# neozenith/sqlite-muninn

Measured on AMD Instinct MI355X. Metric: kNN queries/sec (10k-query batch, k=10, ef=128, 1M x 768 f32 HNSW index) + recall@10, higher is better.
Workload: dtype f32

## Files before the change

### include/muninn_hip.h

```cpp
#ifndef MUNINN_HIP_H
#define MUNINN_HIP_H

#include <stddef.h>
#include <stdint.h>

#ifdef __cplusplus
extern "C" {
#endif

#define MN_ABI_VERSION 2

typedef enum { MN_METRIC_L2 = 0, MN_METRIC_COSINE = 1, MN_METRIC_INNER_PRODUCT = 2 } mn_metric;

typedef enum { MN_ORDER_SSE = 0, MN_ORDER_WAVE = 1 } mn_order;

typedef enum {
    MN_BUILD_SEQUENTIAL = 0,
    MN_BUILD_BATCHED = 1
} mn_build_mode;

typedef struct {
    int64_t id;
    float distance;
} mn_search_result;
// ... 44 lines not shown

int mn_hnsw_get_vector(mn_index *idx, int64_t id, float *out);

int mn_hnsw_node_count(mn_index *idx);
int64_t mn_hnsw_entry_point(mn_index *idx);
int mn_hnsw_max_level(mn_index *idx);
int mn_hnsw_node_level(mn_index *idx, int64_t id);
int mn_hnsw_node_deleted(mn_index *idx, int64_t id);
int mn_hnsw_neighbors(mn_index *idx, int64_t id, int level, int64_t *out, int cap);
int mn_hnsw_load_node(mn_index *idx, int64_t id, const float *vector, int level, int deleted);
int mn_hnsw_load_neighbors(mn_index *idx, int64_t id, int level, const int64_t *nbrs, int n);
int mn_hnsw_set_entry(mn_index *idx, int64_t entry_point, int max_level);

int mn_hnsw_slot_count(mn_index *idx);
int mn_hnsw_export_nodes(mn_index *idx, int64_t *ids, int *levels, int *deleted);
int mn_hnsw_export_vectors(mn_index *idx, float *out);
int mn_hnsw_row_width(mn_index *idx, int level);
int mn_hnsw_export_links(mn_index *idx, int level, int *out, int *width);

int64_t mn_hnsw_take_dirty(mn_index *idx, int64_t *ids, int64_t cap);

int64_t mn_hnsw_edges_of(mn_index *idx, const int64_t *ids, int n, int64_t *out_src, int64_t *out_dst, int *out_level,
                         float *out_dist, int64_t cap);

typedef struct {
    double last_kernel_ms;
    int64_t last_n_dist;
    int64_t last_n_expanded;
    int64_t last_n_overflow;
    int64_t last_n_exact_rows;
    int64_t last_n_rows_lanes4;
    int64_t last_n_rows_lanes8;
    int64_t last_n_rows_lanes16;
} mn_launch_stats;
int mn_hnsw_last_launch(mn_index *idx, mn_launch_stats *out);
typedef struct {
    double search_ms, link_ms;
    int64_t n_dist, n_expanded;
    int64_t batches, nodes;
} mn_build_stats;
int mn_hnsw_build_stats(mn_index *idx, mn_build_stats *out, int reset);
void *mn_dev_malloc(mn_index *idx, size_t bytes);
void mn_dev_free(mn_index *idx, void *p);
int mn_dev_upload(mn_index *idx, void *dst_dev, const void *src_host, size_t bytes);
int mn_dev_download(mn_index *idx, void *dst_host, const void *src_dev, size_t bytes);
int mn_hnsw_bruteforce_topk(mn_index *idx, const float *d_queries, int64_t nq, int k, int64_t *out_ids);

typedef struct {
    int64_t n_queries, n_mfma_queries, n_fallback_queries, n_rescored_rows, n_bound_violations;
    float kernel_ms;
} mn_exact_stats;
int mn_hnsw_search_exact_batch(mn_index *idx, const float *queries, int64_t nq, int k,
                               const int64_t *allow_ids, int64_t n_allow,
                               int64_t *out_ids, float *out_dists, int *out_counts);
int mn_hnsw_search_exact_batch_dev(mn_index *idx, const float *d_queries, int64_t nq, int k,
                                   const int64_t *allow_ids, int64_t n_allow,
                                   int64_t *d_out_ids, float *d_out_dists, int *d_out_counts);
int mn_hnsw_last_exact(mn_index *idx, mn_exact_stats *out);

int mn_hnsw_knn_graph(mn_index *idx, int k, float max_distance, int64_t *out_ids, float *out_dists, int *out_counts);
int mn_hnsw_knn_graph_dev(mn_index *idx, int k, float max_distance, int64_t *d_out_ids, float *d_out_dists, int *d_out_counts);

typedef struct {
    int32_t r1, r2;
    double weight;
} mn_er_edge;
// ... 168 lines not shown
```

### sqlite-muninn_amd/csrc/mn_beam.hpp

```cpp
#pragma once
#include "mn_dist.hpp"

template <bool COH> DEVI int ld_link(const int *p) {
    if (COH)
        return __hip_atomic_load(p, __ATOMIC_RELAXED, __HIP_MEMORY_SCOPE_AGENT);
    return *p;
}
DEVI void st_link(int *p, int v) { __hip_atomic_store(p, v, __ATOMIC_RELAXED, __HIP_MEMORY_SCOPE_AGENT); }


struct WHeap {
    uint2 *l;
    unsigned long long *g;
    int lcap, gcap;
    int size;
    int ovf;
    int sorted = 0;
};

DEVI uint2 hget(const WHeap &h, int i) {
    if (i < h.lcap)
        return h.l[i];
    unsigned long long v = __hip_atomic_load(&h.g[i - h.lcap], __ATOMIC_RELAXED, __HIP_MEMORY_SCOPE_AGENT);
    return make_uint2((unsigned)(v & 0xffffffffull), (unsigned)(v >> 32));
// ... 98 lines not shown
static __device__ unsigned long long mn_phase[MN_PHASE_N];
#define PH_DECL unsigned long long ph_t = __builtin_amdgcn_s_memrealtime()
#define PH_ADD(w, k)                                                                                                             \
    do {                                                                                                                         \
        const unsigned long long ph_n = __builtin_amdgcn_s_memrealtime();                                                        \
        (w).ph[k] += ph_n - ph_t;                                                                                                \
        ph_t = ph_n;                                                                                                             \
    } while (0)
#define PH_CNT(w, k, n) (w).ph[k] += (n)
#else
#define PH_DECL
#define PH_ADD(w, k)
#define PH_CNT(w, k, n)
#endif

struct WaveCtx {
#ifdef MN_PHASE_TIMING
    unsigned long long ph[MN_PHASE_N] = {0, 0, 0, 0, 0, 0, 0, 0, 0, 0, 0, 0, 0, 0, 0, 0};
#endif
    float *tile = nullptr;
    const float *q;
    float qnorm;
    int *scratch;
    unsigned long long n_dist, n_exp;
    int *rlog = nullptr;
    int rcap = 0, nr = 0;
    CoopCtx *coop = nullptr;
    int no_spec_rows = 0;
    int lp_on = 0;
    LoQuery lq = {0.0f, 0.0};
    unsigned long long n_skip = 0;
    int sv_lanes = 0;
    unsigned long long n_l8 = 0, n_l16 = 0;
};
DEVI bool getenv_spec_off(const WaveCtx &w) { return (w.no_spec_rows & 1) != 0; }

DEVI void log_row_read(const MnDevIndex &ix, WaveCtx &w, int node, int level, int lane) {
    if (!w.rlog)
        return;
    if (lane == 0 && w.nr < w.rcap) {
        int *e = w.rlog + (size_t)w.nr * MN_RLOG_INTS;
        e[0] = level == 0 ? node : -(ix.up_off[node] + level - 1) - 2;
        e[1] = (int)0xff800000u;
        e[2] = e[3] = -1;
        e[4] = 0;
    }
    w.nr++;
}
DEVI void log_greedy_detail(WaveCtx &w, float to_beat, int from, int moved_to, int lane) {
    if (!w.rlog)
        return;
    if (lane == 0 && w.nr >= 1 && w.nr <= w.rcap) {
        int *e = w.rlog + (size_t)(w.nr - 1) * MN_RLOG_INTS;
        e[1] = __float_as_int(to_beat);
        e[2] = from;
        e[3] = moved_to;
        e[4] = 1;
    }
}
DEVI void log_row_detail(WaveCtx &w, float worst, unsigned long long could_push, int lane, int kind = 0) {
    if (!w.rlog)
        return;
    if (lane == 0 && w.nr >= 1 && w.nr <= w.rcap) {
        int *e = w.rlog + (size_t)(w.nr - 1) * MN_RLOG_INTS;
        e[1] = __float_as_int(worst);
        e[2] = (int)(unsigned)(could_push & 0xffffffffull);
// ... 104 lines not shown
                    i0 = c0 + 64;
                    fresh = false;
                    continue;
                }
                if (LOG && !WIDE)
                    log_greedy_detail(w, cur_d, i0, -1, lane);
                break;
            }
            int c = __ffsll((long long)better) - 1;
            const float beaten = cur_d;
            const int from = i0;
            cur_d = __shfl(d, c);
            cur = __shfl(myslot, c);
            int pos_of_me = pos;
            __builtin_amdgcn_wave_barrier();
            if (valid)
                w.scratch[rank] = pos_of_me;
            __builtin_amdgcn_wave_barrier();
            i0 = w.scratch[c] + 1;
            i0 = rfl(i0);
            cur = rfl(cur);
            if (LOG && !WIDE)
                log_greedy_detail(w, beaten, from, i0 - 1, lane);
            changed = 1;
            fresh = true;
        }
    }
    return cur;
}

template <int ORDER, int NCH, bool COH = false, bool WIDE = false, bool LOG = false, bool LP = false>
DEVI void beam_layer(const MnDevIndex &ix, WaveCtx &w, WHeap &cand, WHeap &res, unsigned *bitmap, int entry, int level,
                     int ef, int lane) {
    cand.size = 0;
    res.size = 0;
    if (!(ix.has_deleted && ix.deleted[entry])) {
        float d = ctx_distance<ORDER, NCH>(ix, w, entry, 1, lane);
        d = __shfl(d, 0);
        w.n_dist += 1;
        heap_push(cand, entry, d, lane);
        heap_push(res, entry, -d, lane);
        if (lane == 0) {
            int vi = level == 0 ? entry : ix.up_off[entry];
            atomicOr(&bitmap[vi >> 5], 1u << (vi & 31));
        }
    }
    int patience_max = ef / 4;
    if (patience_max < 10)
        patience_max = 10;
    int stale = 0;
    int guard = 0;
    while (cand.size > 0 && guard < (1 << 24)) {
        guard++;
        PH_DECL;
        uint2 c = heap_pop(cand, lane);
        const float cd = u2f(c.x);
        if (res.size >= ef) {
            float worst = -u2f(rflu(hget(res, 1).x));
            if (cd > worst)
                break;
        }
        if (stale >= patience_max && res.size >= ef)
            break;
        const int node = (int)c.y;
        int W;
        const int *row = link_row(ix, node, level, W);
        w.n_exp++;
        if (LOG)
            log_row_read(ix, w, node, level, lane);
        PH_ADD(w, 0);
        PH_CNT(w, 5, 1);
        int improved = 0;
        const int nchunk = WIDE ? (W + 63) >> 6 : 1;
        for (int ch = 0; ch < nchunk; ch++) {
        const int c0 = WIDE ? ch << 6 : 0;
        int nb = (c0 + lane < W) ? ld_link<COH>(row + c0 + lane) : -1;
        bool todo = false;
        if (nb >= 0) {
            int vi = level == 0 ? nb : ix.up_off[nb];
            unsigned bit = 1u << (vi & 31);
            unsigned old = atomicOr(&bitmap[vi >> 5], bit);
            todo = !(old & bit) && !(ix.has_deleted && ix.deleted[nb]);
        }
        unsigned long long m = __ballot(todo);
        int n = __popcll(m);
        PH_ADD(w, 1);
        if (n > 0) {
            int rank = __popcll(m & ((1ull << lane) - 1ull));
            __builtin_amdgcn_wave_barrier();
            if (todo)
                w.scratch[rank] = nb;
            __builtin_amdgcn_wave_barrier();
            int myslot = lane < n ? w.scratch[lane] : 0;
            w.n_dist += n;
            int ne = n;
            if (LP && w.lp_on && res.size >= ef) {
                const float worst0 = -u2f(rflu(hget(res, 1).x));
                const float lb = lo_rows_bound(ix, w.q, w.lq, myslot, n, lane);
                const bool keep = lane < n && !(lb >= worst0);
                const unsigned long long km = __ballot(keep);
                ne = __popcll(km);
                if (ne < n) {
                    w.n_skip += n - ne;
                    const int kr = __popcll(km & ((1ull << lane) - 1ull));
                    __builtin_amdgcn_wave_barrier();
                    if (keep)
                        w.scratch[kr] = myslot;
                    __builtin_amdgcn_wave_barrier();
                    myslot = lane < ne ? w.scratch[lane] : 0;
                }
                PH_ADD(w, 8);
                PH_CNT(w, 9, ne == 0);
                PH_CNT(w, 10, ne >= 1 && ne <= 4);
                PH_CNT(w, 11, ne >= 5 && ne <= 8);
                PH_CNT(w, 12, ne >= 9 && ne <= 16);
                PH_CNT(w, 13, ne > 16);
                PH_CNT(w, 14, 1);
                PH_CNT(w, 15, n);
            }
            float d = 0.0f;
            int quads = 1;
            if (LP && ORDER == MN_ORDER_SSE_V && NCH == 1)
                quads = w.sv_lanes ? w.sv_lanes >> 2 : (ne <= 4 ? 4 : ne <= 8 ? 2 : 1);
            if (LP && quads > 1 && ne > 0) {
                d = rows_distance_spread(ix, w.q, w.qnorm, myslot, ne, lane, quads);
                if (quads == 4)
                    w.n_l16 += ne;
                else
                    w.n_l8 += ne;
            } else if (!LP || ne > 0) {
                int dl = lane;
                if (LP)
                    asm volatile("" : "+v"(dl));
                d = ctx_distance<ORDER, NCH>(ix, w, myslot, ne, dl);
            }
            PH_ADD(w, 2);
            unsigned long long am;
            float worst_log = __builtin_inff();
            if (res.size >= ef) {
                float worst0 = -u2f(rflu(hget(res, 1).x));
                am = __ballot(lane < ne && d < worst0);
                worst_log = worst0;
            } else {
                am = __ballot(lane < ne);
            }
            if (LOG && !WIDE && w.rlog)
                log_row_detail(w, worst_log, __ballot(todo && ((am >> rank) & 1ull)), lane, 2);
            PH_CNT(w, 4, __popcll(am));
            while (am) {
                int i = __ffsll((long long)am) - 1;
                am &= am - 1;
                float di = __shfl(d, i);
                int si = __shfl(myslot, i);
                di = u2f(rflu(f2u(di)));
                si = rfl(si);
                if (res.size < ef) {
                    heap_push(cand, si, di, lane);
                    heap_push(res, si, -di, lane);
                    improved = 1;
                } else {
                    float worst = -u2f(rflu(hget(res, 1).x));
                    if (di < worst) {
                        heap_push(cand, si, di, lane);
                        heap_pop(res, lane);
                        heap_push(res, si, -di, lane);
                        improved = 1;
                    }
                }
            }
            PH_ADD(w, 3);
        } else if (LOG && !WIDE && w.rlog) {
            log_row_detail(w, res.size >= ef ? -u2f(rflu(hget(res, 1).x)) : __builtin_inff(), 0ull, lane, 2);
        }
        }
        stale = improved ? 0 : stale + 1;
    }
    if (guard >= (1 << 24))
        cand.ovf = 1;
#ifdef MN_PHASE_TIMING
    if (lane == 0)
        for (int k = 0; k < MN_PHASE_N; k++) {
            atomicAdd(&mn_phase[k], w.ph[k]);
            w.ph[k] = 0;
        }
#endif
}




#define MN_SA_R 4
#define MN_SA_CAP (64 * MN_SA_R)
#define MN_SA_EACH(X) X(0, k0, v0, s0) X(1, k1, v1, s1) X(2, k2, v2, s2) X(3, k3, v3, s3)
#define MN_SA_DONE ((int)0x80000000)

struct SQueue {
    float k0, k1, k2, k3;
    int v0, v1, v2, v3;
    int rn;
    float wk;
};
// ... 286 lines not shown
```

### sqlite-muninn_amd/csrc/mn_device.hpp

```cpp
#pragma once
#include <hip/hip_runtime.h>
#include <stdint.h>
#include <stdlib.h>

#define MN_WAVE 64

typedef unsigned mn_lo_t;
#define MN_LO_BITS 10
#define MN_LO_CMAX 511
#define MN_LO_LINE_CODES 96
#define MN_LO_LINE_WORDS 32
struct __align__(16) MnLoMeta {
    float scale;
    float resid;
    float xn_lo;
    float xn_hi;
};
#define MN_LO_MIN_LD 192
__host__ __device__ inline bool mn_lo_enabled(int ld) { return ld >= MN_LO_MIN_LD && (ld & 63) == 0; }
__host__ __device__ inline int mn_lo_lines(int ld) { return (ld + MN_LO_LINE_CODES - 1) / MN_LO_LINE_CODES; }
__host__ __device__ inline size_t mn_lo_row_words(int ld) { return (size_t)mn_lo_lines(ld) * MN_LO_LINE_WORDS; }
__host__ __device__ inline int mn_lo_q_floats(int ld) { return mn_lo_enabled(ld) ? mn_lo_lines(ld) * MN_LO_LINE_CODES : ld; }
__host__ __device__ inline int mn_lo_code(unsigned w, int f) { return (int)(w << (32 - MN_LO_BITS * (f + 1))) >> (32 - MN_LO_BITS); }
__host__ __device__ inline unsigned mn_lo_pack(int c0, int c1, int c2) {
    return ((unsigned)c0 & 0x3ffu) | (((unsigned)c1 & 0x3ffu) << 10) | (((unsigned)c2 & 0x3ffu) << 20);
}
constexpr int MN_ORDER_SSE_V = 0;
constexpr int MN_ORDER_WAVE_V = 1;

struct MnDevIndex {
    const float *vectors;
    const float *norms;
    int *links0;
    int *links_up;
    const int *up_off;
    const signed char *levels;
    const unsigned char *deleted;
    unsigned char *dirty;
    const long long *ids;
    int dim, ld, metric, order;
    int W0, WU;
    int M0, MU;
    int WX;
    int n_slots;
    int n_pool_rows;
    int has_deleted;
    const mn_lo_t *vec_lo;
    const MnLoMeta *lo_meta;
};

#define MN_QC 6
struct MnSearchArgs {
    const float *queries;
    const int *query_slots;
    long long nq;
    int k;
    int ef;
    int entry_slot, max_level;
    long long *out_ids;
    float *out_dists;
    int *out_counts;
    int *sel;
    int *nsel;
    int nlev;
    const int *up_bm_index;
    unsigned *bitmap0;
    long long bm0_words;
    unsigned *bitmap_up;
    long long bmu_words;
    uint2 *cand_ovf;
    int cand_gcap;
    uint2 *res_ovf;
    int res_gcap;
    unsigned long long *counters;
    unsigned long long *q_counters;
    int use_tile;
    int lds_bitmap;
    int *readlog;
    int readcap;
    int *nread;
    int lat_tile_rows;
    unsigned lat_tile_off;
    int surv_lanes;
    int no_spec_rows;
};
size_t mn_lds_optin_limit();
bool mn_lds_grant(const void *kernel, size_t bytes);
template <typename K> inline bool mn_lds_grant_for(K kernel, size_t bytes) { return mn_lds_grant(reinterpret_cast<const void *>(kernel), bytes); }
inline int mn_no_spec_rows(long long n_slots, int ld) {
    const char *sr = getenv("MN_SPEC_ROWS");
    const bool big = (size_t)n_slots * ld * sizeof(float) > ((size_t)256 << 20);
    return sr ? (atoi(sr) == 0 ? 1 : 0) : (big ? 0 : 1);
}

#ifndef MN_CAND_LDS
#define MN_CAND_LDS 256
#endif
#ifndef MN_RES_LDS
#define MN_RES_LDS 256
#endif

void mn_module_touch_kernels();
void mn_module_touch_seq();
void mn_module_touch_spec();
void mn_module_touch_build();
void mn_launch_prep_rows(const MnDevIndex &ix, int first_slot, int n, float *norms_out, mn_lo_t *lo_out, MnLoMeta *meta_out,
                         hipStream_t st);
int mn_launch_dist_batch(int metric, int order, const float *d_query, const float *d_rows, long long n, int dim, int ld,
                         float *d_out, hipStream_t st);
size_t mn_dist_batch_lds_bytes(int ld);
size_t mn_search_lds_bytes(int ld, bool tile);
size_t mn_coop_lds_bytes(int ld, bool tile);
size_t mn_spec_commit_min_lds_bytes(int ld);
size_t mn_link_reverse_lds_bytes(int ld, int WX, int nq);
size_t mn_bruteforce_lds_bytes(int ld);
inline size_t mn_row_lds_bytes(int ld) { return (size_t)ld * sizeof(float); }
// ... 71 lines not shown
```

### sqlite-muninn_amd/csrc/mn_dist.hpp

```cpp
#pragma once
#include "mn_device.hpp"

#define DEVI __device__ __forceinline__

DEVI int rfl(int v) { return __builtin_amdgcn_readfirstlane(v); }
DEVI unsigned rflu(unsigned v) { return (unsigned)__builtin_amdgcn_readfirstlane((int)v); }
DEVI float u2f(unsigned u) { return __uint_as_float(u); }
DEVI unsigned f2u(float f) { return __float_as_uint(f); }
DEVI double rfl_f64(double v) {
    const unsigned long long b = (unsigned long long)__double_as_longlong(v);
    return __longlong_as_double((long long)(((unsigned long long)rflu((unsigned)(b >> 32)) << 32) | rflu((unsigned)b)));
}


DEVI float cosine_finish(float dot, float na, float nb) {
    float denom = __fmul_rn(sqrtf(na), sqrtf(nb));
    if (denom < 1e-30f)
        return 1.0f;
    return __fsub_rn(1.0f, __fdiv_rn(dot, denom));
}

DEVI float wave_butterfly(float acc) {
#pragma unroll
    for (int m = 32; m >= 1; m >>= 1)
// ... 609 lines not shown
}

template <int ORDER, int NCH, bool LAT = false>
DEVI float rows_distance(const MnDevIndex &ix, const float *q_lds, float qnorm, int myslot, int n, int lane,
                         float *tile = nullptr, int tile_rows = 0) {
    if (ix.metric == 0) {
        return rows_accumulate<ORDER, NCH, true, LAT>(ix, q_lds, myslot, n, lane, tile, tile_rows);
    }
    float dot = rows_accumulate<ORDER, NCH, false, LAT>(ix, q_lds, myslot, n, lane, tile, tile_rows);
    if (ix.metric == 2)
        return -dot;
    float nb = (lane < n) ? ix.norms[myslot] : 1.0f;
    return cosine_finish(dot, qnorm, nb);
}

DEVI float rows_distance_spread(const MnDevIndex &ix, const float *q_lds, float qnorm, int myslot, int n, int lane, int Q) {
    if (ix.metric == 0)
        return sse_rows_spread<true>(ix, q_lds, myslot, n, lane, Q);
    const float dot = sse_rows_spread<false>(ix, q_lds, myslot, n, lane, Q);
    if (ix.metric == 2)
        return -dot;
    const float nb = (lane < n) ? ix.norms[myslot] : 1.0f;
    return cosine_finish(dot, qnorm, nb);
}


DEVI float lo_deq(int c, float s) { return __fmul_rn((float)c, s); }
DEVI double mn_gamma(int n) {
    const double nu = (double)n * 0x1p-24;
    return nu / (1.0 - nu);
}

template <bool L2, int UB>
DEVI void lo_lines(const uint4 *__restrict__ row, const float *q, float s, int lines, int &k, float &acc) {
    for (; k + UB <= lines; k += UB) {
        uint4 v[UB];
#pragma unroll
        for (int u = 0; u < UB; u++)
            v[u] = row[8 * (k + u)];
        __builtin_amdgcn_sched_barrier(0);
#pragma unroll
        for (int u = 0; u < UB; u++) {
            const float4 qa = *reinterpret_cast<const float4 *>(q + MN_LO_LINE_CODES * (k + u));
            const float4 qb = *reinterpret_cast<const float4 *>(q + MN_LO_LINE_CODES * (k + u) + 4);
            const float4 qc = *reinterpret_cast<const float4 *>(q + MN_LO_LINE_CODES * (k + u) + 8);
            const float qe[12] = {qa.x, qa.y, qa.z, qa.w, qb.x, qb.y, qb.z, qb.w, qc.x, qc.y, qc.z, qc.w};
            const unsigned w4[4] = {v[u].x, v[u].y, v[u].z, v[u].w};
#pragma unroll
            for (int e = 0; e < 12; e++) {
                const float x = lo_deq(mn_lo_code(w4[e / 3], e % 3), s);
                if (L2) {
                    const float d = __fsub_rn(qe[e], x);
                    acc = fmaf(d, d, acc);
                } else {
                    acc = fmaf(qe[e], x, acc);
                }
            }
            __builtin_amdgcn_sched_barrier(0);
        }
    }
}

template <bool L2>
DEVI float lo_rows_accumulate(const MnDevIndex &ix, const float *q_lds, int myslot, float sc, int n, int lane) {
    float mine = 0.0f;
    int ln = lane;
    asm volatile("" : "+v"(ln));
    const int c = ln & 7, r = ln >> 3;
    const int lines = mn_lo_lines(ix.ld);
    const size_t row_words = mn_lo_row_words(ix.ld);
    for (int t = 0; t < n; t += 8) {
        const int rr = t + r < n ? t + r : n - 1;
        const int sl = __shfl(myslot, rr);
        const float s = __shfl(sc, rr);
        const uint4 *row = reinterpret_cast<const uint4 *>(ix.vec_lo + (size_t)sl * row_words) + c;
        const float *q = q_lds + 12 * c;
        float acc = 0.0f;
        int k = 0;
        lo_lines<L2, 8>(row, q, s, lines, k, acc);
        lo_lines<L2, 2>(row, q, s, lines, k, acc);
        lo_lines<L2, 1>(row, q, s, lines, k, acc);
        acc += quad_xor1(acc);
        acc += quad_xor2(acc);
        acc += __int_as_float(__builtin_amdgcn_ds_swizzle(__float_as_int(acc), 0x101F));
        const float got = __shfl(acc, ((ln - t) & 7) << 3);
        if (ln >= t && ln < t + 8)
            mine = got;
    }
    return mine;
}

struct LoQuery {
    double qs_lo;
    double qn_hi;
};
DEVI LoQuery lo_query(float qsq, int ld) {
    LoQuery lq;
    lq.qs_lo = sqrt((double)qsq) * (1.0 - 0x1p-40);
    const double lost = (double)ld * 0x1p-149;
    lq.qn_hi = sqrt(((double)qsq + lost) / (1.0 - 2.0 * mn_gamma(ld + 8))) * (1.0 + 0x1p-40);
    return lq;
}

DEVI float lo_lower_bound(int metric, float A, const MnLoMeta &m, const LoQuery &lq, int ld) {
    const double a = A, r = m.resid, g = mn_gamma(ld + 8), u = 0x1p-24;
    if (!(fabs(a) <= 3.0e38) || !(r <= 3.0e38))
        return -__builtin_inff();
    double lb;
    if (metric == 0) {
        const double l = (double)sqrtf((float)(fmax(a - (double)ld * 0x1p-147, 0.0) * (1.0 - 4.0 * g))) * (1.0 - 0x1p-21) - 2.0 * r;
        lb = l > 0.0 ? l * l * (1.0 - 4.0 * g) : 0.0;
    } else {
        const double e = 2.0 * (lq.qn_hi * (r + g * (2.0 * (double)m.xn_hi + r)) + (double)ld * 0x1p-147);
        if (metric == 2) {
            lb = -(a + e);
        } else {
            const double den = lq.qs_lo * (double)m.xn_lo * (1.0 - 8.0 * u);
            if (!(den >= 1e-28))
                return -__builtin_inff();
            lb = 1.0 - fmax(a + e, 0.0) / den * (1.0 + 4.0 * u);
        }
    }
    lb -= fabs(lb) * 0x1p-20 + 0x1p-120;
    const float f = __double2float_rd(lb);
    return f == f ? f : -__builtin_inff();
}

template <int ORDER>
DEVI float lds_self_norm(const float *q_lds, int dim, int ld, int lane) {
    if (ORDER == MN_ORDER_SSE_V) {
        float v = sse_row<false>(q_lds, q_lds, dim, lane);
        return __shfl(v, 0);
    }
    return wave_row_generic<false>(q_lds, q_lds, ld, lane);
}

DEVI float lo_rows_bound(const MnDevIndex &ix, const float *q_lds, const LoQuery &lq, int myslot, int n, int lane) {
    MnLoMeta m = {1.0f, __builtin_inff(), 0.0f, 0.0f};
    if (lane < n)
        m = ix.lo_meta[myslot];
    const float A = ix.metric == 0 ? lo_rows_accumulate<true>(ix, q_lds, myslot, m.scale, n, lane)
                                   : lo_rows_accumulate<false>(ix, q_lds, myslot, m.scale, n, lane);
    return lane < n ? lo_lower_bound(ix.metric, A, m, lq, ix.ld) : -__builtin_inff();
}
```

### sqlite-muninn_amd/csrc/mn_index_int.hpp

```cpp
#pragma once
#include "../../include/muninn_hip.h"
#include "mn_comm.hpp"
#include "mn_device.hpp"
#include "mn_guard.hpp"
#include "mn_host.hpp"

#include <algorithm>
#include <cstdlib>
#include <cstring>
#include <string>
#include <vector>

void set_err(const char *fmt, ...) __attribute__((format(printf, 1, 2)));
#define HIPCHK(expr) MN_HIPCHK(set_err, expr)

template <typename T> struct DevBuf {
    T *p = nullptr;
    size_t cap = 0;
    DevBuf() = default;
    DevBuf(const DevBuf &) = delete;
    DevBuf &operator=(const DevBuf &) = delete;
    ~DevBuf() { release(); }
    int reserve(size_t n, bool keep, hipStream_t st, int fill_byte = -1, size_t want = 0) {
        if (n <= cap)
// ... 70 lines not shown
    bool dev_links_all = false;
    std::vector<std::pair<int, int>> h_dirty_rows;
    std::vector<float> load_vecs;
    int load_first = -1;
    DevBuf<unsigned> ws_bm0, ws_bmu;
    DevBuf<uint2> ws_cand, ws_res;
    DevBuf<float> ws_q, ws_outd;
    DevBuf<long long> ws_outi;
    DevBuf<int> ws_outc, ws_qslots, ws_sel, ws_nsel, ws_upidx;
    DevBuf<int> lk_target, lk_src, lk_counters, lk_count, lk_fill, lk_binoff, lk_touched, lk_bins, lk_newrows;
    DevBuf<int> lk_rec, lk_rec_all, lk_cls;
    DevBuf<unsigned long long> ws_counters;
    DevBuf<int> ws_state;
    DevBuf<int> er_slot, er_level, er_nbr;
    DevBuf<float> er_dist;
    DevBuf<int> ws_readlog, ws_nread, ws_ncommit, d_stamp0, d_stampU, d_sidx0, d_sidxU, d_saved_rows, d_pre_act, d_pre_cnt, d_pre_row, d_spec_why;
    int spec_epoch = 0;
    std::vector<int> staged;
    DevBuf<int> d_staged;
    DevBuf<int> sh_sel, sh_nsel, sh_gcnt;
    DevBuf<int> ws_chlog;
    bool want_chlog = false;
    std::vector<int> h_chlog;
    std::vector<unsigned char> h_stale;
    int n_stale = 0;
    unsigned char *pin = nullptr;
    size_t pin_cap = 0;
    DevBuf<unsigned long long> sh_ovf;
    int sh_ovf_pending = 0;
    DevBuf<long long> sh_gids;
    DevBuf<float> sh_gd;
    long long last_spec_searched = 0;
    bool broken = false;
    mn_launch_stats last = {0, 0, 0, 0, 0, 0, 0, 0};
    mn_exact_stats last_exact = {0, 0, 0, 0, 0, 0.0f};
};

int use_device(mn_index *x);
MnDevIndex dev_view(mn_index *x);
int ht_find(const mn_index *x, int64_t id);
void ht_grow(mn_index *x);
int random_level(mn_index *x);
int host_add_node(mn_index *x, int64_t id, int level, int deleted);
int64_t first_table_full(const mn_index *x, int64_t n);
void mark_stale(mn_index *x, int slot);
struct InsertUndo {
    int first, node_count, max_level, n_pool_rows, old_cap = 0, grew_at = -1;
    unsigned rng;
    int64_t entry_id;
    std::vector<int> old_ht;
};
void undo_insert(mn_index *x, InsertUndo &u);
int sync_meta(mn_index *x);
int upload_vectors(mn_index *x, int first, const float *vecs, int n, bool src_on_device = false);
int pull_links(mn_index *x);
int push_links(mn_index *x);
unsigned char *pin_reserve(mn_index *x, size_t need);
#define MN_PIN_META 0
#define MN_PIN_IN 64
#define MN_PIN_OUT 96
#define MN_PIN_VEC 256
inline size_t pin_log_off(const mn_index *x) { return (MN_PIN_VEC + (size_t)x->ld * sizeof(float) + 63) & ~(size_t)63; }
inline size_t pin_insert_bytes(const mn_index *x) {
    return pin_log_off(x) + ((size_t)1 + (size_t)MN_CHLOG_CAP * MN_CHLOG_INTS) * sizeof(int);
}

inline int cand_gcap(int ef) { return 16 * ef + 1024; }
// ... 10 lines not shown
```

### sqlite-muninn_amd/csrc/mn_index_search.hip

```cpp
#include "mn_index_int.hpp"

#include <cstdio>


static int reserve_search_ws(mn_index *x, int64_t nq, int ef) {
    hipStream_t st = x->stream;
    if (x->ws_bm0.reserve((size_t)nq * bm0_words(x->n_slots), false, st)) return -1;
    if (x->ws_cand.reserve((size_t)nq * cand_gcap(ef), false, st)) return -1;
    if (x->ws_res.reserve((size_t)nq * res_gcap(ef), false, st)) return -1;
    if (x->ws_counters.reserve(8, false, st)) return -1;
    return 0;
}

int prepare_search_ws(mn_index *x, int64_t nq, int ef, MnSearchArgs &a, bool zero_counters, bool lds_bitmap_ok) {
    hipStream_t st = x->stream;
    a.bm0_words = bm0_words(x->n_slots);
    a.cand_gcap = cand_gcap(ef);
    a.res_gcap = res_gcap(ef);
    if (reserve_search_ws(x, nq, ef))
        return -1;
    a.lds_bitmap = lds_bitmap_ok && nq <= 128 &&
                   (long long)mn_search_lds_bytes(x->ld, true) + 1024 + a.bm0_words * (long long)sizeof(unsigned) <= 64 * 1024 &&
                   !(getenv("MN_COOP") && atoi(getenv("MN_COOP")) == 0) && !(getenv("MN_LDS_BITMAP") && atoi(getenv("MN_LDS_BITMAP")) == 0);
    if (!a.lds_bitmap)
        HIPCHK(hipMemsetAsync(x->ws_bm0.p, 0, (size_t)nq * a.bm0_words * sizeof(unsigned), st));
    if (zero_counters)
        HIPCHK(hipMemsetAsync(x->ws_counters.p, 0, 8 * sizeof(unsigned long long), st));
    a.bitmap0 = x->ws_bm0.p;
    a.cand_ovf = x->ws_cand.p;
    a.res_ovf = x->ws_res.p;
    a.counters = x->ws_counters.p;
    a.bitmap_up = nullptr;
    a.bmu_words = 0;
    a.no_spec_rows = mn_no_spec_rows(x->n_slots, x->ld);
#ifdef MN_SSE_TILE_PATH
    const char *e = getenv("MN_SSE_TILE");
    a.use_tile = e ? atoi(e) : 1;
#else
    a.use_tile = 0;
#endif
    return 0;
}

void last_from_counters(mn_index *x, const unsigned long long *c, bool timed) {
    float ms = 0;
    if (!timed)
        x->last.last_kernel_ms = 0.0f;
    else if (hipEventElapsedTime(&ms, x->ev0, x->ev1) == hipSuccess)
        x->last.last_kernel_ms = ms;
    x->last.last_n_dist = (int64_t)c[0];
    x->last.last_n_expanded = (int64_t)c[1];
    x->last.last_n_overflow = (int64_t)c[2];
    x->last.last_n_exact_rows = (int64_t)(c[0] - c[3]);
    x->last.last_n_rows_lanes8 = (int64_t)c[4];
    x->last.last_n_rows_lanes16 = (int64_t)c[5];
    x->last.last_n_rows_lanes4 = x->last.last_n_exact_rows - (int64_t)(c[4] + c[5]);
}

int fetch_counters(mn_index *x) {
    unsigned long long c[8];
    if (!x->ws_counters.p)
        return 0;
    HIPCHK(hipMemcpyAsync(c, x->ws_counters.p, sizeof(c), hipMemcpyDeviceToHost, x->stream));
    HIPCHK(hipStreamSynchronize(x->stream));
    last_from_counters(x, c, true);
    return 0;
}

static int search_batch_dev_impl(mn_index *x, const float *d_queries, int64_t nq, int k, int ef, int64_t *d_ids, float *d_dists,
                                 int *d_counts, unsigned long long *q_counters) {
    if (use_device(x))
        return -1;
    if (nq <= 0)
        return 0;
    if (k <= 0) {
        set_err("mn_hnsw_search: k must be > 0");
        return -1;
    }
    if (ef < k)
        ef = k;
    hipStream_t st = x->stream;
    if (x->entry_id == -1 || x->node_count == 0) {
        HIPCHK(hipMemsetAsync(d_counts, 0, (size_t)nq * sizeof(int), st));
        HIPCHK(hipMemsetAsync(d_ids, 0xFF, (size_t)nq * k * sizeof(int64_t), st));
        HIPCHK(hipMemsetAsync(d_dists, 0, (size_t)nq * k * sizeof(float), st));
        return 0;
    }
    if (push_links(x) || sync_meta(x))
        return -1;
// ... 68 lines not shown

extern "C" int mn_hnsw_sync(mn_index *x) try {
    if (use_device(x))
        return -1;
    HIPCHK(hipStreamSynchronize(x->stream));
    return check_sharded_overflow(x);
} MN_GUARD_END(set_err, MN_NOTHING, -1)

static int search_small(mn_index *x, const float *queries, int64_t nq, int k, int ef, int64_t *out_ids, float *out_dists,
                        int *out_counts) {
    hipStream_t st = x->stream;
    const size_t qb = (size_t)nq * x->dim * sizeof(float), ib = (size_t)nq * k * sizeof(int64_t), db = (size_t)nq * k * sizeof(float);
    const size_t cb = ((size_t)nq * sizeof(int) + 7) & ~(size_t)7;
    const size_t o_ids = (qb + 15) & ~(size_t)15, o_d = o_ids + ib, o_c = (o_d + db + 7) & ~(size_t)7, o_cnt = o_c + cb;
    const size_t need = o_cnt + (size_t)nq * MN_QC * sizeof(unsigned long long);
    if (push_links(x) || sync_meta(x))
        return -1;
    if (!pin_reserve(x, need)) {
        set_err("mn_hnsw_search: cannot allocate %zu bytes of pinned host memory", need);
        return -1;
    }
    HIPCHK(hipStreamSynchronize(st));
    memcpy(x->pin, queries, qb);
    unsigned long long *qc = reinterpret_cast<unsigned long long *>(x->pin + o_cnt);
    if (search_batch_dev_impl(x, (const float *)x->pin, nq, k, ef, (int64_t *)(x->pin + o_ids), (float *)(x->pin + o_d),
                              (int *)(x->pin + o_c), qc))
        return -1;
    const bool launched = x->entry_id != -1 && x->node_count > 0;
    HIPCHK(hipStreamSynchronize(st));
    memcpy(out_ids, x->pin + o_ids, ib);
    memcpy(out_dists, x->pin + o_d, db);
    memcpy(out_counts, x->pin + o_c, (size_t)nq * sizeof(int));
    if (launched) {
        unsigned long long tot[MN_QC] = {0, 0, 0, 0, 0, 0};
        for (int64_t q = 0; q < nq; q++)
            for (int i = 0; i < MN_QC; i++)
                tot[i] += qc[q * MN_QC + i];
        last_from_counters(x, tot, false);
        x->last_on_host = true;
        if (x->last.last_n_overflow) {
            set_err("mn_hnsw_search: %lld queries exceeded heap workspace", (long long)x->last.last_n_overflow);
            return -1;
        }
    }
    return 0;
}

template <typename F>
static int with_staged_io(mn_index *x, const float *queries, size_t nq, int k, int64_t *out_ids, float *out_dists, int *out_counts,
                          F &&dev_face) {
    hipStream_t st = x->stream;
    if (queries && x->ws_q.reserve(nq * x->dim, false, st)) return -1;
    if (x->ws_outi.reserve(nq * k, false, st)) return -1;
    if (x->ws_outd.reserve(nq * k, false, st)) return -1;
    if (x->ws_outc.reserve(nq, false, st)) return -1;
    if (queries)
        HIPCHK(hipMemcpyAsync(x->ws_q.p, queries, nq * x->dim * sizeof(float), hipMemcpyHostToDevice, st));
    if (dev_face())
        return -1;
    HIPCHK(hipMemcpyAsync(out_ids, x->ws_outi.p, nq * k * sizeof(int64_t), hipMemcpyDeviceToHost, st));
    HIPCHK(hipMemcpyAsync(out_dists, x->ws_outd.p, nq * k * sizeof(float), hipMemcpyDeviceToHost, st));
    HIPCHK(hipMemcpyAsync(out_counts, x->ws_outc.p, nq * sizeof(int), hipMemcpyDeviceToHost, st));
    HIPCHK(hipStreamSynchronize(st));
    return 0;
}

extern "C" int mn_hnsw_search_batch(mn_index *x, const float *queries, int64_t nq, int k, int ef, int64_t *out_ids,
// ... 341 lines not shown
```

### sqlite-muninn_amd/csrc/mn_kernels.hip

```cpp
#include "mn_device.hpp"
#include <cstdio>
#include <cstdlib>
#include <mutex>
#include <unordered_map>

#include "mn_dist.hpp"
#include "mn_dispatch.hpp"


DEVI double wave_sum_f64(double v) {
#pragma unroll
    for (int m = 32; m >= 1; m >>= 1)
        v += __shfl_xor(v, m);
    return v;
}

template <int ORDER>
__global__ void __launch_bounds__(64)
    k_prep_rows(MnDevIndex ix, int first_slot, int n, float *norms_out, mn_lo_t *lo_out, MnLoMeta *meta_out) {
    extern __shared__ float lds[];
    const int lane = threadIdx.x;
    int slot = first_slot + blockIdx.x;
    if (blockIdx.x >= n)
        return;
// ... 163 lines not shown
    if (BUILD) {
        qslot = a.query_slots[qi];
        qsrc = ix.vectors + (size_t)qslot * ix.ld;
    } else {
        qsrc = a.queries + (size_t)qi * ix.dim;
    }
    for (int i = lane; i < qf; i += 64)
        q[i] = i < ix.dim ? qsrc[i] : 0.0f;
    __builtin_amdgcn_s_waitcnt(0);
    __builtin_amdgcn_wave_barrier();

    WaveCtx w;
    w.q = q;
    w.tile = (ORDER == MN_ORDER_SSE_V && a.use_tile) ? tile : nullptr;
    w.scratch = scratch;
    w.n_dist = 0;
    w.n_exp = 0;
    w.qnorm = 0.0f;
    if (ix.metric == 1)
        w.qnorm = BUILD ? ix.norms[qslot] : lds_self_norm<ORDER>(q, ix.dim, ix.ld, lane);
    if (coop) {
        w.coop = coop;
        w.no_spec_rows = a.no_spec_rows;
        if (lane == 0)
            *coop->qnorm = w.qnorm;
    }
    if (LP) {
        w.lq = lo_query(ix.metric == 1 ? w.qnorm : lds_self_norm<ORDER>(q, ix.dim, ix.ld, lane), ix.ld);
        w.lp_on = w.lq.qn_hi <= 1.0e300;
        w.lq.qs_lo = rfl_f64(w.lq.qs_lo);
        w.lq.qn_hi = rfl_f64(w.lq.qn_hi);
        w.qnorm = u2f(rflu(f2u(w.qnorm)));
        w.sv_lanes = a.surv_lanes;
    }
    if (BUILD && a.readlog) {
        w.rlog = a.readlog + (size_t)qi * a.readcap * MN_RLOG_INTS;
        w.rcap = a.readcap;
    }

    WHeap cand, res;
    cand.l = cand_l;
    cand.lcap = MN_CAND_LDS;
    cand.g = reinterpret_cast<unsigned long long *>(a.cand_ovf + (size_t)qi * a.cand_gcap);
    cand.gcap = a.cand_gcap;
    cand.size = 0;
    cand.ovf = 0;
    res.l = res_l;
    res.lcap = MN_RES_LDS;
    res.g = reinterpret_cast<unsigned long long *>(a.res_ovf + (size_t)qi * a.res_gcap);
    res.gcap = a.res_gcap;
    res.size = 0;
    res.ovf = 0;

    unsigned *bm0 = lds_bitmap ? lds_bitmap : a.bitmap0 + (size_t)qi * a.bm0_words;
    int cur = a.entry_slot;

    if (!BUILD) {
        for (int l = a.max_level; l > 0; l--)
            cur = greedy_layer<ORDER, NCH, false, WIDE>(ix, w, cur, l, lane);
        if (LAT)
            beam_layer_auto<ORDER, NCH, false, WIDE>(ix, w, cand, res, bm0, a.bm0_words, cur, 0, a.ef, lane);
        else
            beam_layer<ORDER, NCH, false, WIDE, false, LP>(ix, w, cand, res, bm0, cur, 0, a.ef, lane);
        int count = res.size;
        int outn = count < a.k ? count : a.k;
        for (int i = count - 1; i >= 0; i--) {
// ... 21 lines not shown
                bm = a.bitmap_up + ((size_t)a.up_bm_index[qi] * a.max_level + (l - 1)) * a.bmu_words;
            if (LAT)
                beam_layer_auto<ORDER, NCH, false, WIDE, true>(ix, w, cand, res, bm, l > 0 ? a.bmu_words : a.bm0_words, cur, l, a.ef, lane);
            else
                beam_layer<ORDER, NCH, false, WIDE>(ix, w, cand, res, bm, cur, l, a.ef, lane);
            const int M_max = (l == 0) ? ix.M0 : ix.MU;
            int count = res.size;
            int keep = count < M_max ? count : M_max;
            int *sel = a.sel + ((size_t)qi * a.nlev + l) * ix.M0;
            int first = cur;
            for (int i = count - 1; i >= 0; i--) {
                uint2 it = res_take(res, i, count, lane);
                if (i < keep && lane == 0)
                    sel[i] = (int)it.y;
                if (i == 0)
                    first = (int)it.y;
            }
            if (lane == 0)
                a.nsel[qi * a.nlev + l] = keep;
            if (count > 0)
                cur = first;
        }
    }
    if (lane == 0) {
        if (BUILD && a.readlog)
            a.nread[qi] = LAT ? w.nr : a.readcap + 1;
        if (a.q_counters) {
            a.q_counters[(size_t)qi * MN_QC + 0] = w.n_dist;
            a.q_counters[(size_t)qi * MN_QC + 1] = w.n_exp;
            a.q_counters[(size_t)qi * MN_QC + 2] = (cand.ovf || res.ovf) ? 1ull : 0ull;
            a.q_counters[(size_t)qi * MN_QC + 3] = w.n_skip;
            a.q_counters[(size_t)qi * MN_QC + 4] = w.n_l8;
            a.q_counters[(size_t)qi * MN_QC + 5] = w.n_l16;
        } else {
            atomicAdd(&a.counters[0], w.n_dist);
            atomicAdd(&a.counters[1], w.n_exp);
            if (cand.ovf || res.ovf)
                atomicAdd(&a.counters[2], 1ull);
            if (LP && w.n_skip)
                atomicAdd(&a.counters[3], w.n_skip);
            if (LP && w.n_l8)
                atomicAdd(&a.counters[4], w.n_l8);
            if (LP && w.n_l16)
                atomicAdd(&a.counters[5], w.n_l16);
        }
    }
}

template <int ORDER, int NCH, bool BUILD, bool WIDE = false, bool LP = false>
__global__ void __launch_bounds__(64) k_beam(MnDevIndex ix, MnSearchArgs a) {
    extern __shared__ __align__(16) unsigned char smem[];
    if ((long long)blockIdx.x >= a.nq)
        return;
    beam_query<ORDER, NCH, BUILD, WIDE, false, LP>(ix, a, blockIdx.x, threadIdx.x, smem, nullptr);
}

#define MN_COOP_WAVES 8
template <int ORDER, int NCH, bool BUILD, bool WIDE = false>
__global__ void __launch_bounds__(MN_COOP_WAVES * 64) k_beam_coop(MnDevIndex ix, MnSearchArgs a, size_t base_lds) {
    extern __shared__ __align__(16) unsigned char smem[];
    if ((long long)blockIdx.x >= a.nq)
        return;
    const int lane = threadIdx.x & 63;
    CoopCtx c;
    c.n = reinterpret_cast<int *>(smem + base_lds);
    c.qnorm = reinterpret_cast<float *>(c.n + 1);
    c.list = c.n + 4;
    c.dist = reinterpret_cast<float *>(c.list + 64);
    c.nw = blockDim.x >> 6;
    c.wv = threadIdx.x >> 6;
    if (a.lat_tile_rows > 0) {
        c.tile = reinterpret_cast<float *>(smem + a.lat_tile_off) + (size_t)c.wv * mn_lat_tile_floats(ix.ld, a.lat_tile_rows);
        c.tile_rows = a.lat_tile_rows;
    }
    unsigned *lbm = nullptr;
    if (!BUILD && a.lds_bitmap) {
        lbm = reinterpret_cast<unsigned *>(smem + base_lds) + 4 + 64 + 64;
// ... 85 lines not shown
    }
    if (getenv("MN_LAT_DEBUG"))
        fprintf(stderr, "[mn] k_beam_coop: distance tile of %d rows per wavefront, %zu bytes of LDS\n", a.lat_tile_rows, tot);
    hipLaunchKernelGGL((k_beam_coop<ORDER, NCH, BUILD, WIDE>), dim3((unsigned)a.nq), dim3(MN_COOP_WAVES * 64), tot, st, ix, a, base);
}

template <int ORDER, int NCH>
static void launch_beam(const MnDevIndex &ix, const MnSearchArgs &a, bool build, hipStream_t st) {
    dim3 grid((unsigned)a.nq), block(64);
    size_t lds = mn_search_lds_bytes(ix.ld, ORDER == MN_ORDER_SSE_V && a.use_tile);
    const bool wide = ix.WX > 64;
    const char *co = getenv("MN_COOP");
    if (a.nq <= 128 && !(co && atoi(co) == 0)) {
        const size_t base = (lds + 15) & ~(size_t)15;
        const size_t tot = mn_coop_lds_bytes(ix.ld, ORDER == MN_ORDER_SSE_V && a.use_tile) +
                           (!build && a.lds_bitmap ? (size_t)a.bm0_words * sizeof(unsigned) : 0);
        if (wide) {
            if (build)
                launch_coop<ORDER, NCH, true, true>(ix, a, base, tot, st);
            else
                launch_coop<ORDER, NCH, false, true>(ix, a, base, tot, st);
        } else if (build)
            launch_coop<ORDER, NCH, true, false>(ix, a, base, tot, st);
        else
            launch_coop<ORDER, NCH, false, false>(ix, a, base, tot, st);
        return;
    }
    const char *lp = getenv("MN_LOWPREC_FILTER");
    if (!build && ix.vec_lo && ix.lo_meta && !(lp && atoi(lp) == 0)) {
        MnSearchArgs al = a;
        const char *sv = getenv("MN_SURVIVOR_LANES");
        const int svl = sv ? atoi(sv) : 0;
        al.surv_lanes = (svl == 4 || svl == 8 || svl == 16) ? svl : 0;
        if (wide)
            hipLaunchKernelGGL((k_beam<ORDER, NCH, false, true, true>), grid, block, lds, st, ix, al);
        else
            hipLaunchKernelGGL((k_beam<ORDER, NCH, false, false, true>), grid, block, lds, st, ix, al);
        return;
    }
    if (wide) {
        if (build)
            hipLaunchKernelGGL((k_beam<ORDER, NCH, true, true>), grid, block, lds, st, ix, a);
        else
            hipLaunchKernelGGL((k_beam<ORDER, NCH, false, true>), grid, block, lds, st, ix, a);
    } else if (build)
        hipLaunchKernelGGL((k_beam<ORDER, NCH, true>), grid, block, lds, st, ix, a);
    else
        hipLaunchKernelGGL((k_beam<ORDER, NCH, false>), grid, block, lds, st, ix, a);
}

int mn_launch_search(const MnDevIndex &ix, const MnSearchArgs &a, bool build, hipStream_t st) {
    if (a.nq <= 0)
        return 0;
    if (ix.order == MN_ORDER_SSE_V) {
        const char *qe = getenv("MN_SSE_QUAD");
        if (MN_SSE_QUAD2 > 0 && (ix.dim >> 4) >= MN_SSE_QUAD2 && !(qe && atoi(qe) == 0))
            launch_beam<MN_ORDER_SSE_V, 1>(ix, a, build, st);
        else
            launch_beam<MN_ORDER_SSE_V, 0>(ix, a, build, st);
        return 0;
    }
    mn_for_wave_walk(ix.ld, [&](auto O, auto N) { launch_beam<O(), N()>(ix, a, build, st); });
    return 0;
}


// ... 106 lines not shown
```

### sqlite-muninn_amd/hnsw.py

```python
from __future__ import annotations

import ctypes as C
import os

import numpy as np

from .build import LIB

METRIC = {"l2": 0, "cosine": 1, "inner_product": 2}
ORDER_SSE, ORDER_WAVE = 0, 1
BUILD_SEQUENTIAL, BUILD_BATCHED = 0, 1

_f32p = np.ctypeslib.ndpointer(np.float32, flags="C_CONTIGUOUS")
_i64p = np.ctypeslib.ndpointer(np.int64, flags="C_CONTIGUOUS")
_i32p = np.ctypeslib.ndpointer(np.int32, flags="C_CONTIGUOUS")


class MuninnHipError(RuntimeError):
    pass


class _Result(C.Structure):
    _fields_ = [("id", C.c_int64), ("distance", C.c_float)]


class LaunchStats(C.Structure):
    _fields_ = [("last_kernel_ms", C.c_double), ("last_n_dist", C.c_int64), ("last_n_expanded", C.c_int64),
                ("last_n_overflow", C.c_int64), ("last_n_exact_rows", C.c_int64),
                ("last_n_rows_lanes4", C.c_int64), ("last_n_rows_lanes8", C.c_int64), ("last_n_rows_lanes16", C.c_int64)]


class ExactStats(C.Structure):
    _fields_ = [("n_queries", C.c_int64), ("n_mfma_queries", C.c_int64), ("n_fallback_queries", C.c_int64),
                ("n_rescored_rows", C.c_int64), ("n_bound_violations", C.c_int64), ("kernel_ms", C.c_float)]


class BuildStats(C.Structure):
    _fields_ = [("search_ms", C.c_double), ("link_ms", C.c_double), ("n_dist", C.c_int64), ("n_expanded", C.c_int64),
                ("batches", C.c_int64), ("nodes", C.c_int64)]


class ErEdge(C.Structure):
    _fields_ = [("r1", C.c_int32), ("r2", C.c_int32), ("weight", C.c_double)]


class ErStats(C.Structure):
    _fields_ = [("n_candidates", C.c_int64), ("n_edges", C.c_int64), ("n_jw_short", C.c_int64), ("n_jw_long", C.c_int64),
                ("blocking_ms", C.c_double), ("candidates_ms", C.c_double), ("score_ms", C.c_double)]


_u8p = np.ctypeslib.ndpointer(np.uint8, flags="C_CONTIGUOUS")
_f64p = np.ctypeslib.ndpointer(np.float64, flags="C_CONTIGUOUS")

ER_SYMBOLS = [
    ("mn_er_jaro_winkler", C.c_int, [C.c_int64, _u8p, _i64p, C.c_int64, _i32p, _i32p, C.c_int, _f64p]),
    ("mn_er_candidates", C.c_int64, [C.c_int, C.c_int, _i64p, _i64p, _f32p, _i32p, C.c_double, C.c_int, _i32p, _i32p, _f64p]),
    ("mn_er_score", C.c_int64, [C.c_int64, _i32p, _i32p, _f64p, C.c_int, _u8p, _i64p, C.c_void_p, C.c_int, C.c_double, C.c_double,
                                C.c_int, C.c_void_p]),
    ("mn_hnsw_er_edges", C.c_int64, [C.c_void_p, C.c_int, _i64p, _u8p, _i64p, C.c_void_p, C.c_int, C.c_double, C.c_double, C.c_double,
                                     C.c_int, C.c_int, C.c_void_p, C.POINTER(ErStats)]),
]

# ... 483 lines not shown
```

Before: 593,200.

## Speculatively prefetch next beam node's link row and visited bits during heap updates

In the low-precision-filter beam search at level 0, each row update predicts which candidate will be expanded next: the heap top, or the nearest newly admitted neighbour. It then loads that node's link row and sets its visited bits while the heap pushes are still running, overlapping the gather latency with heap maintenance. On a misprediction the speculatively set bits are cleared with atomicAnd and a fence, and the row is reloaded, adding rollback cost and code complexity. Smaller changes move a shuffle of the scale into the unrolled loop, make the lo_meta load unconditional, and add a mispredict counter to the stats.

```diff
diff --git a/include/muninn_hip.h b/include/muninn_hip.h
--- a/include/muninn_hip.h
+++ b/include/muninn_hip.h
@@ -100,6 +100,7 @@
     int64_t last_n_rows_lanes4;
     int64_t last_n_rows_lanes8;
     int64_t last_n_rows_lanes16;
+    int64_t last_n_mispredict;
 } mn_launch_stats;
 int mn_hnsw_last_launch(mn_index *idx, mn_launch_stats *out);
 typedef struct {
diff --git a/sqlite-muninn_amd/csrc/mn_beam.hpp b/sqlite-muninn_amd/csrc/mn_beam.hpp
--- a/sqlite-muninn_amd/csrc/mn_beam.hpp
+++ b/sqlite-muninn_amd/csrc/mn_beam.hpp
@@ -154,6 +154,8 @@
     unsigned long long n_skip = 0;
     int sv_lanes = 0;
     unsigned long long n_l8 = 0, n_l16 = 0;
+    int pf_on = 0;
+    unsigned long long n_mis = 0;
 };
 DEVI bool getenv_spec_off(const WaveCtx &w) { return (w.no_spec_rows & 1) != 0; }
 
@@ -324,6 +326,58 @@
 template <int ORDER, int NCH, bool COH = false, bool WIDE = false, bool LOG = false, bool LP = false>
 DEVI void beam_layer(const MnDevIndex &ix, WaveCtx &w, WHeap &cand, WHeap &res, unsigned *bitmap, int entry, int level,
                      int ef, int lane) {
+    constexpr bool PF = LP && !WIDE && !COH && !LOG;
+    int pf_node = -1;
+    int pf_nb = -1;
+    unsigned pf_old = 0;
+    unsigned char pf_del = 0;
+    auto pf_probe = [&]() {
+        asm volatile("" : "+v"(pf_nb));
+        if (pf_nb >= 0) {
+            const int vi = level == 0 ? pf_nb : ix.up_off[pf_nb];
+            if (ix.has_deleted)
+                pf_del = ix.deleted[pf_nb];
+            pf_old = atomicOr(&bitmap[vi >> 5], 1u << (vi & 31));
+        }
+    };
+    auto pf_predict = [&](unsigned long long am, float d, int myslot) {
+        int ln = lane;
+        asm volatile("" : "+v"(ln));
+        const bool in_am = ((am >> ln) & 1ull) != 0;
+        unsigned long long lt = am;
+        int pred = -1;
+        if (cand.size > 0) {
+            const uint2 rt = hget(cand, 1);
+            const float kT = u2f(rflu(rt.x));
+            lt = __ballot(in_am && d < kT);
+            if (!__ballot(in_am && !(d > kT)))
+                pred = (int)rflu(rt.y);
+        }
+        if (pred < 0 && lt) {
+            float best = __builtin_inff();
+            int bl = -1;
+            bool tie = false;
+            while (lt) {
+                const int j = rfl(__ffsll((long long)lt) - 1);
+                lt &= lt - 1;
+                const float y = __int_as_float(__builtin_amdgcn_readlane(__float_as_int(d), j));
+                if (y < best) {
+                    best = y;
+                    bl = j;
+                    tie = false;
+                } else if (y == best) {
+                    tie = true;
+                }
+            }
+            if (bl >= 0 && !tie)
+                pred = __builtin_amdgcn_readlane(myslot, bl);
+        }
+        if (pred >= 0) {
+            pf_node = pred;
+            pf_nb = ln < ix.W0 ? ix.links0[(size_t)pred * ix.W0 + ln] : -1;
+        }
+        return pred >= 0;
+    };
     cand.size = 0;
     res.size = 0;
     if (!(ix.has_deleted && ix.deleted[entry])) {
@@ -366,13 +420,42 @@
         const int nchunk = WIDE ? (W + 63) >> 6 : 1;
         for (int ch = 0; ch < nchunk; ch++) {
         const int c0 = WIDE ? ch << 6 : 0;
-        int nb = (c0 + lane < W) ? ld_link<COH>(row + c0 + lane) : -1;
+        int nb;
         bool todo = false;
+        if constexpr (PF) {
+            PH_CNT(w, 6, pf_node == node ? 1 : 0);
+            if (pf_node != node) {
+                if (pf_node >= 0) {
+                    w.n_mis++;
+                    if (pf_nb >= 0) {
+                        const int vi = level == 0 ? pf_nb : ix.up_off[pf_nb];
+                        const unsigned bit = 1u << (vi & 31);
+                        if (!(pf_old & bit))
+                            atomicAnd(&bitmap[vi >> 5], ~bit);
+                    }
+                    __builtin_amdgcn_fence(__ATOMIC_RELEASE, "agent");
+                    __builtin_amdgcn_s_waitcnt(0);
+                }
+                pf_nb = (lane < W) ? ld_link<COH>(row + lane) : -1;
+                pf_probe();
+            }
+            pf_node = -1;
+            nb = pf_nb;
+            if (nb >= 0) {
+                const int vi = level == 0 ? nb : ix.up_off[nb];
+                todo = !(pf_old & (1u << (vi & 31))) && !(ix.has_deleted && pf_del);
+            }
+            pf_nb = -1;
+            pf_old = 0;
+            pf_del = 0;
+        } else {
+        nb = (c0 + lane < W) ? ld_link<COH>(row + c0 + lane) : -1;
         if (nb >= 0) {
             int vi = level == 0 ? nb : ix.up_off[nb];
             unsigned bit = 1u << (vi & 31);
             unsigned old = atomicOr(&bitmap[vi >> 5], bit);
             todo = !(old & bit) && !(ix.has_deleted && ix.deleted[nb]);
+        }
         }
         unsigned long long m = __ballot(todo);
         int n = __popcll(m);
@@ -439,6 +522,12 @@
             if (LOG && !WIDE && w.rlog)
                 log_row_detail(w, worst_log, __ballot(todo && ((am >> rank) & 1ull)), lane, 2);
             PH_CNT(w, 4, __popcll(am));
+            bool probe_due = false;
+            if constexpr (PF) {
+                if (w.pf_on && level == 0 && res.size >= ef)
+                    probe_due = pf_predict(am, d, myslot);
+                PH_CNT(w, 7, probe_due ? 1 : 0);
+            }
             while (am) {
                 int i = __ffsll((long long)am) - 1;
                 am &= am - 1;
@@ -459,6 +548,16 @@
                         improved = 1;
                     }
                 }
+                if constexpr (PF) {
+                    if (probe_due) {
+                        pf_probe();
+                        probe_due = false;
+                    }
+                }
+            }
+            if constexpr (PF) {
+                if (probe_due)
+                    pf_probe();
             }
             PH_ADD(w, 3);
         } else if (LOG && !WIDE && w.rlog) {
diff --git a/sqlite-muninn_amd/csrc/mn_device.hpp b/sqlite-muninn_amd/csrc/mn_device.hpp
--- a/sqlite-muninn_amd/csrc/mn_device.hpp
+++ b/sqlite-muninn_amd/csrc/mn_device.hpp
@@ -49,7 +49,7 @@
     const MnLoMeta *lo_meta;
 };
 
-#define MN_QC 6
+#define MN_QC 7
 struct MnSearchArgs {
     const float *queries;
     const int *query_slots;
@@ -82,6 +82,7 @@
     int lat_tile_rows;
     unsigned lat_tile_off;
     int surv_lanes;
+    int beam_prefetch;
     int no_spec_rows;
 };
 size_t mn_lds_optin_limit();
diff --git a/sqlite-muninn_amd/csrc/mn_dist.hpp b/sqlite-muninn_amd/csrc/mn_dist.hpp
--- a/sqlite-muninn_amd/csrc/mn_dist.hpp
+++ b/sqlite-muninn_amd/csrc/mn_dist.hpp
@@ -665,13 +665,14 @@
 }
 
 template <bool L2, int UB>
-DEVI void lo_lines(const uint4 *__restrict__ row, const float *q, float s, int lines, int &k, float &acc) {
+DEVI void lo_lines(const uint4 *__restrict__ row, const float *q, float sc, int rr, int lines, int &k, float &acc) {
     for (; k + UB <= lines; k += UB) {
         uint4 v[UB];
 #pragma unroll
         for (int u = 0; u < UB; u++)
             v[u] = row[8 * (k + u)];
         __builtin_amdgcn_sched_barrier(0);
+        const float s = __shfl(sc, rr);
 #pragma unroll
         for (int u = 0; u < UB; u++) {
             const float4 qa = *reinterpret_cast<const float4 *>(q + MN_LO_LINE_CODES * (k + u));
@@ -705,14 +706,13 @@
     for (int t = 0; t < n; t += 8) {
         const int rr = t + r < n ? t + r : n - 1;
         const int sl = __shfl(myslot, rr);
-        const float s = __shfl(sc, rr);
         const uint4 *row = reinterpret_cast<const uint4 *>(ix.vec_lo + (size_t)sl * row_words) + c;
         const float *q = q_lds + 12 * c;
         float acc = 0.0f;
         int k = 0;
-        lo_lines<L2, 8>(row, q, s, lines, k, acc);
-        lo_lines<L2, 2>(row, q, s, lines, k, acc);
-        lo_lines<L2, 1>(row, q, s, lines, k, acc);
+        lo_lines<L2, 8>(row, q, sc, rr, lines, k, acc);
+        lo_lines<L2, 2>(row, q, sc, rr, lines, k, acc);
+        lo_lines<L2, 1>(row, q, sc, rr, lines, k, acc);
         acc += quad_xor1(acc);
         acc += quad_xor2(acc);
         acc += __int_as_float(__builtin_amdgcn_ds_swizzle(__float_as_int(acc), 0x101F));
@@ -769,9 +769,7 @@
 }
 
 DEVI float lo_rows_bound(const MnDevIndex &ix, const float *q_lds, const LoQuery &lq, int myslot, int n, int lane) {
-    MnLoMeta m = {1.0f, __builtin_inff(), 0.0f, 0.0f};
-    if (lane < n)
-        m = ix.lo_meta[myslot];
+    const MnLoMeta m = ix.lo_meta[myslot];
     const float A = ix.metric == 0 ? lo_rows_accumulate<true>(ix, q_lds, myslot, m.scale, n, lane)
                                    : lo_rows_accumulate<false>(ix, q_lds, myslot, m.scale, n, lane);
     return lane < n ? lo_lower_bound(ix.metric, A, m, lq, ix.ld) : -__builtin_inff();
diff --git a/sqlite-muninn_amd/csrc/mn_index_int.hpp b/sqlite-muninn_amd/csrc/mn_index_int.hpp
--- a/sqlite-muninn_amd/csrc/mn_index_int.hpp
+++ b/sqlite-muninn_amd/csrc/mn_index_int.hpp
@@ -126,7 +126,7 @@
     DevBuf<float> sh_gd;
     long long last_spec_searched = 0;
     bool broken = false;
-    mn_launch_stats last = {0, 0, 0, 0, 0, 0, 0, 0};
+    mn_launch_stats last = {0, 0, 0, 0, 0, 0, 0, 0, 0};
     mn_exact_stats last_exact = {0, 0, 0, 0, 0, 0.0f};
 };
 
diff --git a/sqlite-muninn_amd/csrc/mn_index_search.hip b/sqlite-muninn_amd/csrc/mn_index_search.hip
--- a/sqlite-muninn_amd/csrc/mn_index_search.hip
+++ b/sqlite-muninn_amd/csrc/mn_index_search.hip
@@ -55,6 +55,7 @@
     x->last.last_n_rows_lanes8 = (int64_t)c[4];
     x->last.last_n_rows_lanes16 = (int64_t)c[5];
     x->last.last_n_rows_lanes4 = x->last.last_n_exact_rows - (int64_t)(c[4] + c[5]);
+    x->last.last_n_mispredict = (int64_t)c[6];
 }
 
 int fetch_counters(mn_index *x) {
@@ -189,7 +190,7 @@
     memcpy(out_dists, x->pin + o_d, db);
     memcpy(out_counts, x->pin + o_c, (size_t)nq * sizeof(int));
     if (launched) {
-        unsigned long long tot[MN_QC] = {0, 0, 0, 0, 0, 0};
+        unsigned long long tot[8] = {0, 0, 0, 0, 0, 0, 0, 0};
         for (int64_t q = 0; q < nq; q++)
             for (int i = 0; i < MN_QC; i++)
                 tot[i] += qc[q * MN_QC + i];
diff --git a/sqlite-muninn_amd/csrc/mn_kernels.hip b/sqlite-muninn_amd/csrc/mn_kernels.hip
--- a/sqlite-muninn_amd/csrc/mn_kernels.hip
+++ b/sqlite-muninn_amd/csrc/mn_kernels.hip
@@ -219,6 +219,7 @@
         w.lq.qn_hi = rfl_f64(w.lq.qn_hi);
         w.qnorm = u2f(rflu(f2u(w.qnorm)));
         w.sv_lanes = a.surv_lanes;
+        w.pf_on = a.beam_prefetch;
     }
     if (BUILD && a.readlog) {
         w.rlog = a.readlog + (size_t)qi * a.readcap * MN_RLOG_INTS;
@@ -306,6 +307,7 @@
             a.q_counters[(size_t)qi * MN_QC + 3] = w.n_skip;
             a.q_counters[(size_t)qi * MN_QC + 4] = w.n_l8;
             a.q_counters[(size_t)qi * MN_QC + 5] = w.n_l16;
+            a.q_counters[(size_t)qi * MN_QC + 6] = w.n_mis;
         } else {
             atomicAdd(&a.counters[0], w.n_dist);
             atomicAdd(&a.counters[1], w.n_exp);
@@ -317,6 +319,8 @@
                 atomicAdd(&a.counters[4], w.n_l8);
             if (LP && w.n_l16)
                 atomicAdd(&a.counters[5], w.n_l16);
+            if (LP && w.n_mis)
+                atomicAdd(&a.counters[6], w.n_mis);
         }
     }
 }
@@ -468,6 +472,8 @@
         const char *sv = getenv("MN_SURVIVOR_LANES");
         const int svl = sv ? atoi(sv) : 0;
         al.surv_lanes = (svl == 4 || svl == 8 || svl == 16) ? svl : 0;
+        const char *pf = getenv("MN_BEAM_PREFETCH");
+        al.beam_prefetch = !(pf && atoi(pf) == 0);
         if (wide)
             hipLaunchKernelGGL((k_beam<ORDER, NCH, false, true, true>), grid, block, lds, st, ix, al);
         else
diff --git a/sqlite-muninn_amd/hnsw.py b/sqlite-muninn_amd/hnsw.py
--- a/sqlite-muninn_amd/hnsw.py
+++ b/sqlite-muninn_amd/hnsw.py
@@ -27,7 +27,8 @@
 class LaunchStats(C.Structure):
     _fields_ = [("last_kernel_ms", C.c_double), ("last_n_dist", C.c_int64), ("last_n_expanded", C.c_int64),
                 ("last_n_overflow", C.c_int64), ("last_n_exact_rows", C.c_int64),
-                ("last_n_rows_lanes4", C.c_int64), ("last_n_rows_lanes8", C.c_int64), ("last_n_rows_lanes16", C.c_int64)]
+                ("last_n_rows_lanes4", C.c_int64), ("last_n_rows_lanes8", C.c_int64), ("last_n_rows_lanes16", C.c_int64),
+                ("last_n_mispredict", C.c_int64)]
 
 
 class ExactStats(C.Structure):
```

New measurement: 594,700, median of 6. No clear change (+0.2%).
